# thierrydumas/autoencoder_based_image_compression

Measured on AMD Instinct MI355X. Metric: Mpixels/s encode+decode (Kodak 768x512 luma), bitstream bit-exact, higher is better.
Workload: dtype f32; 1 GPU; kodak_512x768_luma_batch24_per_gpu_bin_width_1.0_lossless_roundtrip; height=512, width=768, truncated_unary_length=10, idx_map_exception=67, parallelism=single GPU, coder=device, 64 maps per wavefront, encode + decode + compare

## Files before the change

autoencoder_based_image_compression_amd/csrc/hip/coder_simd.hip:

```cpp
#include <hip/hip_runtime.h>
#include <stdint.h>

#include <mutex>

#include "../coder/lean_step.h"
#include "eae_hip.h"

int eae_coder_generic_encode(uint32_t n_maps, uint32_t map_size, const int16_t* symbols, uint8_t L, const double* probs,
                             const int32_t* prob_row, uint8_t* streams, uint64_t stride, uint32_t* bac_bits,
                             uint32_t* bypass_bits, int32_t* status, int32_t* stage, int only_status, hipStream_t stream);
int eae_coder_generic_decode(uint32_t n_maps, uint32_t map_size, int16_t* out, uint8_t L, const double* probs,
                             const int32_t* prob_row, const uint8_t* streams, uint64_t stride, const uint32_t* bac_bits,
                             const uint32_t* bypass_bits, int32_t* status, int32_t* stage, int only_status, hipStream_t stream);

#ifndef EAE_RES_BINARISE
#define EAE_RES_BINARISE 47
#endif
#ifndef EAE_RES_ENCODE_CORE
#define EAE_RES_ENCODE_CORE 55
#endif
#ifndef EAE_RES_EMIT
#define EAE_RES_EMIT 39
#endif
#ifndef EAE_RES_DECODE_CORE
#define EAE_RES_DECODE_CORE 55
#endif
#ifndef EAE_RES_DEBINARISE
#define EAE_RES_DEBINARISE 23
#endif
#ifndef EAE_RES_DEBINARISE_STAGED
#define EAE_RES_DEBINARISE_STAGED 39
#endif
#ifndef EAE_RES_DECODE_CORE_CHUNKED
#define EAE_RES_DECODE_CORE_CHUNKED 63
#endif
#ifndef EAE_DECODE_TOPUP_ZEROS
#define EAE_KEEP_VGPR_FREE_(n) asm volatile("; v" #n " reserved: the last register of the allocation holds no operand" ::: "v" #n)
#define EAE_KEEP_LAST_VGPR_FREE(n) EAE_KEEP_VGPR_FREE_(n)
#else
#define EAE_KEEP_LAST_VGPR_FREE(n)
#endif

namespace {

using namespace eae_core;
using namespace eae_lean;


#ifndef EAE_SIMD_PRIO
#define EAE_SIMD_PRIO 3
#endif

constexpr int32_t RETRY = -100;
constexpr uint32_t kMaxFastL = 32;
constexpr uint32_t kRecordPad = 12;
constexpr uint32_t kRing = 32;
constexpr uint32_t kBypassStage = 512;
constexpr uint32_t kDebinariseStage = 1024;
constexpr uint32_t kEmitWords = 224;

struct SimdParams {
    uint32_t n_maps, map_size, L, dcap;
    uint32_t rcap;
    const int16_t* symbols;
    int16_t* decoded;
    const double* probs;
    const int32_t* prob_row;
    uint8_t* streams;
    uint64_t stride;
    uint32_t* bac_bits;
    uint32_t* bypass_bits;
    int32_t* status;
    int32_t* stage;
    uint8_t* decisions;
    uint32_t* ndec;
    uint32_t* records;
    uint8_t* prefixes;
    uint32_t chunk, nchunks;
    uint32_t* group_steps;
    uint2* enc_state;
    uint4* emit_state;
    uint32_t* avail_bits;
    uint4* dec_state;
    uint2* dec_state2;
};

__host__ __device__ inline uint32_t chunk_span(uint32_t steps, uint32_t nchunks) {
    const uint32_t span = ((steps + nchunks - 1u) / nchunks + 63u) & ~63u;
    return span ? span : 64u;
}

__device__ __forceinline__ uint32_t wave_exclusive_scan(uint32_t v, uint32_t& total) {
    int inc = (int)v;
    inc += __builtin_amdgcn_update_dpp(0, inc, 0x111, 0xF, 0xF, false);
    inc += __builtin_amdgcn_update_dpp(0, inc, 0x112, 0xF, 0xF, false);
    inc += __builtin_amdgcn_update_dpp(0, inc, 0x114, 0xF, 0xF, false);
    inc += __builtin_amdgcn_update_dpp(0, inc, 0x118, 0xF, 0xF, false);
    inc += __builtin_amdgcn_update_dpp(0, inc, 0x142, 0xA, 0xF, false);
    inc += __builtin_amdgcn_update_dpp(0, inc, 0x143, 0xC, 0xF, false);
    total = (uint32_t)__builtin_amdgcn_readlane(inc, 63);
    return (uint32_t)inc - v;
}
__device__ __forceinline__ int wave_exclusive_max(int v) {
    int m = __builtin_amdgcn_update_dpp(-1, v, 0x138, 0xF, 0xF, false);
#define EAE_MAX_STEP(ctrl_, rows_)                                                        \
    {                                                                                     \
        const int o_ = __builtin_amdgcn_update_dpp(-1, m, ctrl_, rows_, 0xF, false);      \
        m = o_ > m ? o_ : m;                                                              \
    }
    EAE_MAX_STEP(0x111, 0xF)
    EAE_MAX_STEP(0x112, 0xF)
    EAE_MAX_STEP(0x114, 0xF)
    EAE_MAX_STEP(0x118, 0xF)
    EAE_MAX_STEP(0x142, 0xA)
    EAE_MAX_STEP(0x143, 0xC)
#undef EAE_MAX_STEP
    return m;
}
__device__ __forceinline__ uint32_t wave_max(uint32_t v) {
#pragma unroll
    for (int d = 32; d >= 1; d >>= 1) {
        const uint32_t o = __shfl_xor(v, d, 64);
        v = o > v ? o : v;
    }
    return v;
}

__global__ __launch_bounds__(64) void binarise_kernel(const SimdParams p) {
    EAE_KEEP_LAST_VGPR_FREE(EAE_RES_BINARISE);
    __shared__ unsigned long long ybuf[40];
    const uint32_t m = blockIdx.x, lane = threadIdx.x;
    const int32_t row = p.prob_row ? p.prob_row[m] : (int32_t)m;
    if (row < 0) {
        if (lane == 0) { p.ndec[m] = 0; p.bac_bits[m] = 0; p.bypass_bits[m] = 0; p.status[m] = 0; if (p.stage) p.stage[m] = 0; }
        return;
    }
    const uint32_t L = p.L;
    const int16_t* in = p.symbols + (size_t)m * p.map_size;
    uint8_t* dec = p.decisions + (size_t)(m >> 6) * 64u * p.dcap + (size_t)(m & 63u) * 8u;
    unsigned long long* ystream = reinterpret_cast<unsigned long long*>(p.streams + (uint64_t)m * p.stride + p.stride / 2);
    const uint32_t size_bits = round_up_to_byte(required_bits(p.map_size, L));
    uint32_t jbase = 0, bbase = 0;
    bool overflow = false;
    if (lane < 40) ybuf[lane] = 0;
    for (uint32_t t = 0; t < p.map_size; t += 64) {
        const uint32_t i = t + lane;
        const bool valid = i < p.map_size;
        const int s = valid ? (int)in[i] : 0;
        const uint32_t a = (uint32_t)(s < 0 ? -s : s);
        const uint32_t ones = a < L ? a : L;
        const uint32_t nd = valid ? ones + (a < L ? 1u : 0u) : 0u;
        unsigned long long bb = 0;
        uint32_t nb = 0;
        if (valid && a >= L) {
            const uint32_t v = a - L + 1u;
            const uint32_t n = count_nb_bits(v) - 1u;
            bb = ((1ull << n) - 1ull) | ((unsigned long long)(n ? rev16(v - (1u << n)) >> (16u - n) : 0u) << (n + 1u));
            nb = 2u * n + 1u;
        }
        if (valid && s != 0) {
            bb |= (unsigned long long)(s > 0 ? 1u : 0u) << nb;
            nb++;
        }
        uint32_t both_tot;
        const uint32_t both = wave_exclusive_scan(nd | (nb << 16), both_tot);
        const uint32_t jo = both & 0xFFFFu, bo = both >> 16, jtot = both_tot & 0xFFFFu, btot = both_tot >> 16;
        for (uint32_t q = 0; q < nd; q++) {
            const uint32_t j = jbase + jo + q;
            dec[(size_t)(j >> 3) * 512u + (j & 7u)] = (uint8_t)((q << 1) | (q < ones ? 1u : 0u));
        }
        if (nb) {
            const uint32_t pos = (bbase & 63u) + bo;
            atomicOr(&ybuf[pos >> 6], bb << (pos & 63u));
            if ((pos & 63u) + nb > 64u) atomicOr(&ybuf[(pos >> 6) + 1u], bb >> (64u - (pos & 63u)));
        }
        if (bbase + btot > size_bits) overflow = true;
        if (overflow) break;
        const uint32_t nfull = ((bbase & 63u) + btot) >> 6;
        const unsigned long long mine = lane < 40 ? ybuf[lane] : 0ull;
        const unsigned long long carry = ybuf[nfull];
        if (lane < nfull) ystream[(bbase >> 6) + lane] = mine;
        if (lane < 40) ybuf[lane] = lane == 0 ? carry : 0ull;
        jbase += jtot;
        bbase += btot;
    }
    if (lane == 0) {
        if (!overflow && (bbase & 63u)) ystream[bbase >> 6] = ybuf[0];
        p.ndec[m] = jbase;
        p.bypass_bits[m] = bbase;
        p.bac_bits[m] = 0;
        p.status[m] = overflow ? RETRY : 0;
        if (p.stage) p.stage[m] = 0;
    }
}

extern __shared__ double lds_dyn[];

template <bool CHUNKED>
__global__ __launch_bounds__(64) void bac_encode_core_kernel(const SimdParams p) {
    EAE_KEEP_LAST_VGPR_FREE(EAE_RES_ENCODE_CORE);
    __builtin_amdgcn_s_setprio(EAE_SIMD_PRIO);
    const uint32_t lane = threadIdx.x;
    const uint32_t m = blockIdx.x * 64u + lane;
    const bool in_range = m < p.n_maps;
    const int32_t row = in_range ? (p.prob_row ? p.prob_row[m] : (int32_t)m) : -1;
    const bool live = in_range && row >= 0 && p.status[m] == 0;
    const uint32_t L = p.L;
    double* probs = lds_dyn;
    bool retry = false;
    if (live)
        for (uint32_t k = 0; k < L; k++) {
            const double pk = p.probs[(size_t)row * L + k];
            probs[k * 64u + lane] = scale_probability(pk);
            if (!(pk > 0. && pk < 1.)) retry = true;
        }
    const uint32_t nd = live && !retry ? p.ndec[m] : 0u;
    uint32_t steps = wave_max(nd);
    const uint32_t nd_all = ~wave_max(~(nd ? nd : 0xFFFFFFFFu));
    const uint8_t* dec = p.decisions + (size_t)blockIdx.x * 64u * p.dcap + (size_t)lane * 8u;
    uint32_t* rec = p.records + (size_t)(in_range ? m : 0u) * p.rcap;
    Interval s = interval_init();
    uint32_t j_first = 0;
    if (CHUNKED) {
        if (p.chunk == 0u) { if (lane == 0u) p.group_steps[blockIdx.x] = steps; }
        else steps = p.group_steps[blockIdx.x];
        const uint32_t span = chunk_span(steps, p.nchunks);
        j_first = p.chunk * span < steps ? p.chunk * span : steps;
        steps = j_first + span < steps ? j_first + span : steps;
        if (p.chunk != 0u && in_range) { const uint2 st = p.enc_state[m]; s.lo = st.x; s.hc = st.y; }
    }
    const uint32_t last_round = (steps ? steps - 1u : 0u) >> 3;
    auto decisions_of = [&](uint32_t round) __attribute__((always_inline)) {
        return *reinterpret_cast<const uint2*>(dec + (size_t)(round < last_round ? round : last_round) * 512u);
    };
    uint32_t* const sink = rec + p.dcap + 8u;
    const uint32_t nd_here = CHUNKED ? (nd < steps ? nd : steps) : nd;
    auto round_of_eight = [&](const uint2& d, uint32_t jb) __attribute__((always_inline)) {
        const unsigned long long d8 = (unsigned long long)d.x | ((unsigned long long)d.y << 32);
        auto probability = [&](uint32_t q) __attribute__((always_inline)) {
// ... 348 lines not shown
                    const bool need = rcount <= 32u;
                    rwin |= (unsigned long long)(need ? wnext : 0u) << (need ? 32u - rcount : 0u);
                    rcount += need ? 32u : 0u;
                    rword += need ? 1u : 0u;
                    const DecodeStep d = decode_step(s, code32, pk);
                    const uint32_t k = d.take < left ? d.take : left;
                    uint32_t bits = (uint32_t)((rwin >> 1) >> (63u - k));
                    const uint32_t ext = d.take - k;
                    bits = (bits << ext) | ((bits & 1u) ? ((1u << ext) - 1u) : 0u);
                    rwin <<= k;
                    rcount -= k;
                    left -= k;
                    code32 = shift_code(code32, d, bits);
                    const bool done = !d.one || unary + 1u == L;
                    if (done) prefix[i] = (uint8_t)(d.one ? L : unary);
                    i += done ? 1u : 0u;
                    unary = done ? 0u : unary + 1u;
                    pk = done ? p0 : pspec;
                }
            }
            }
            if (!__any(i < size && (!CHUNKED || final_chunk || (begun && left >= kStepMargin)))) break;
        }
    }
    if (CHUNKED && size && !final_chunk) {
        p.dec_state[m] = make_uint4(s.lo, s.hc, code32, begun ? nbac - left : kNotStarted);
        p.dec_state2[m] = make_uint2(unary, i);
    }
    if (live && retry) p.status[m] = RETRY;
#ifdef EAE_HWID_PROBE
    {
        const unsigned int hw1 = __builtin_amdgcn_s_getreg(((32 - 1) << 11) | (0 << 6) | 4);
        const unsigned int xcc1 = __builtin_amdgcn_s_getreg(((4 - 1) << 11) | (0 << 6) | 20);
        if (lane == 0) {
            atomicAdd(&g_hwid_probe[0], 1u);
            if (((hw1 ^ probe_hw0) & 0xFFFFu) != 0u || xcc1 != probe_xcc0) {
                atomicAdd(&g_hwid_probe[1], 1u);
                g_hwid_probe[2] = probe_hw0; g_hwid_probe[3] = probe_xcc0; g_hwid_probe[4] = hw1; g_hwid_probe[5] = xcc1;
            }
        }
    }
#endif
}

#ifdef EAE_HWID_PROBE
extern "C" int eae_hip_debug_hwid_probe(unsigned int* out8) {
    return (int)hipMemcpyFromSymbol(out8, HIP_SYMBOL(g_hwid_probe), 8 * sizeof(unsigned int));
}
#endif

template <bool STAGED>
__global__ __launch_bounds__(64) void debinarise_kernel(const SimdParams p) {
    if (STAGED) { EAE_KEEP_LAST_VGPR_FREE(EAE_RES_DEBINARISE_STAGED); } else { EAE_KEEP_LAST_VGPR_FREE(EAE_RES_DEBINARISE); }
    __shared__ uint32_t ytile[80];
    const uint32_t m = blockIdx.x, lane = threadIdx.x;
    const int32_t row = p.prob_row ? p.prob_row[m] : (int32_t)m;
    if (lane == 0 && p.ndec) p.ndec[m] = 0u;
    if (row < 0 || p.status[m] != 0) {
        if (row >= 0 && p.status[m] == RETRY && lane == 0 && p.ndec) p.ndec[m] = 1u;
        return;
    }
    const uint32_t L = p.L, size = p.map_size;
    const uint32_t nbyp = p.bypass_bits[m];
    const uint32_t* gbyp = reinterpret_cast<const uint32_t*>(p.streams + (uint64_t)m * p.stride + p.stride / 2);
    const uint32_t ywords = (nbyp + 31u) >> 5;
    const uint8_t* prefix = p.prefixes + (size_t)m * size;
    const int16_t* expected = p.symbols ? p.symbols + (size_t)m * size : nullptr;
    int16_t* out = p.decoded ? p.decoded + (size_t)m * size : nullptr;
    uint32_t ybase = 0;
    bool bad = false, differ = false;
    __shared__ uint32_t ystage[STAGED ? kBypassStage + 80u : 1u];
    __shared__ uint8_t pstage[STAGED ? kDebinariseStage : 1u];
    __shared__ int16_t estage[STAGED ? kDebinariseStage : 1u];
    if (STAGED) {
        const uint32_t have = ywords < kBypassStage ? ywords : kBypassStage, last = ywords ? ywords - 1u : 0u;
        for (uint32_t k = 0; k < have; k += 512u) {
            uint32_t v[8];
#pragma unroll
            for (uint32_t u = 0; u < 8; u++) {
                const uint32_t w = k + u * 64u + lane;
                v[u] = gbyp[w < last ? w : last];
            }
#pragma unroll
            for (uint32_t u = 0; u < 8; u++) {
                const uint32_t w = k + u * 64u + lane;
                if (w < kBypassStage) ystage[w] = w < ywords ? v[u] : 0u;
            }
        }
        for (uint32_t w = have + lane; w < kBypassStage + 80u; w += 64u) ystage[w] = 0u;
    }
    for (uint32_t t = 0; t < size; t += 64u) {
        if (STAGED && (t & (kDebinariseStage - 1u)) == 0u) {
            const uint32_t last = size - 1u;
            __syncthreads();
            for (uint32_t k = 0; k < kDebinariseStage && t + k < size; k += 512u) {
                uint8_t pv[8];
                int16_t ev[8];
#pragma unroll
                for (uint32_t u = 0; u < 8; u++) {
                    const uint32_t i = t + k + u * 64u + lane, at_i = i < last ? i : last;
                    pv[u] = prefix[at_i];
                    ev[u] = expected ? expected[at_i] : (int16_t)0;
                }
#pragma unroll
                for (uint32_t u = 0; u < 8; u++) {
                    pstage[k + u * 64u + lane] = pv[u];
                    estage[k + u * 64u + lane] = ev[u];
                }
            }
            __syncthreads();
        }
        const uint32_t w0 = ybase >> 5;
        const bool in_stage = STAGED && (ywords <= kBypassStage ? w0 <= kBypassStage : w0 + 80u <= kBypassStage);
        if (!in_stage) {
            ytile[lane] = w0 + lane < ywords ? gbyp[w0 + lane] : 0u;
            if (lane < 16u) ytile[64u + lane] = w0 + 64u + lane < ywords ? gbyp[w0 + 64u + lane] : 0u;
        }
        const uint32_t* const window = in_stage ? ystage + w0 : ytile;
        auto bits_at = [&](uint32_t pos) {
            const uint32_t rel = pos - (w0 << 5), q = rel >> 5, sh = rel & 31u;
            const unsigned long long two = (unsigned long long)window[q] | ((unsigned long long)window[q + 1u] << 32);
            return (uint32_t)(two >> sh);
        };
        const uint32_t i = t + lane;
        const bool valid = i < size;
        uint32_t a = valid ? (uint32_t)(STAGED ? pstage[i & (kDebinariseStage - 1u)] : prefix[i]) : 0u;
        const bool nonzero = a != 0u;
        uint32_t ntot;
        uint32_t at = wave_exclusive_scan(nonzero ? 1u : 0u, ntot);
        uint32_t extra = 0;
        unsigned long long escapes = __ballot(valid && a == L);
        uint32_t extra_tot = 0;
        while (escapes) {
            const int e = __builtin_ctzll(escapes);
            escapes &= escapes - 1ull;
            const uint32_t pos = ybase + (uint32_t)__builtin_amdgcn_readlane((int)at, e) + extra_tot;
            const uint32_t w = bits_at(pos);
            const uint32_t nn = (uint32_t)__builtin_ctz(~w | 0x80000000u);
            if (nn > 16u || pos + 2u * nn + 1u > nbyp) { bad = true; break; }
            const uint32_t suffix = nn ? __builtin_bitreverse32(bits_at(pos + nn + 1u)) >> (32u - nn) : 0u;
            const uint32_t value = (L + ((suffix + (1u << nn) - 1u) & 0xFFFFu)) & 0xFFFFu;
            const uint32_t len = 2u * nn + 1u;
            if ((int)lane == e) a = value;
            if ((int)lane >= e) extra += len;
            extra_tot += len;
        }
        if (bad) break;
        const uint32_t spos = ybase + at + extra;
        if (nonzero && spos >= nbyp) bad = true;
        if (__any(bad)) { bad = true; break; }
        int v = (int)(int16_t)a;
        if (nonzero && !(bits_at(spos) & 1u)) v = -v;
        if (valid) {
            if (out) out[i] = (int16_t)v;
            if (expected && (STAGED ? estage[i & (kDebinariseStage - 1u)] : expected[i]) != (int16_t)v) differ = true;
        }
        ybase += ntot + extra_tot;
    }
    const bool any_differ = __any(differ);
    if (lane == 0) {
        if (bad) { p.status[m] = RETRY; if (p.ndec) p.ndec[m] = 1u; }
        else if (expected && any_differ) p.status[m] = MISMATCH;
    }
}

__global__ __launch_bounds__(64) void compare_kernel(const SimdParams p) {
    const uint32_t m = blockIdx.x, lane = threadIdx.x;
    if (p.ndec[m] == 0u) return;
    const int32_t row = p.prob_row ? p.prob_row[m] : (int32_t)m;
    if (row < 0 || p.status[m] != 0) return;
    const int16_t* a = p.symbols + (size_t)m * p.map_size;
    const int16_t* b = p.decoded + (size_t)m * p.map_size;
    int differ = 0;
    for (uint32_t i = lane; i < p.map_size; i += 64) differ |= (a[i] != b[i]);
    if (__any(differ) && lane == 0) p.status[m] = MISMATCH;
}

#ifdef EAE_EXPERIMENTAL_CODER
constexpr uint32_t kPipeRecords = 64u;
constexpr uint32_t kPipeSpinLimit = 1u << 21;
constexpr uint32_t kPipeDone = 0x80000000u, kPipeBad = 0x40000000u;

#define EAE_PIPE_ORDER() asm volatile("s_waitcnt lgkmcnt(0)" ::: "memory")

constexpr size_t pipe_lds_bytes(uint32_t L) {
    return ((size_t)L + 1u) * 64u * sizeof(double) + ((size_t)kPipeRecords + kRing) * 64u * sizeof(uint32_t) + (8u + 4u * 64u) * sizeof(uint32_t);
}

#ifndef EAE_RES_PIPE
#define EAE_RES_PIPE 63
#endif

#ifdef EAE_PIPE_PROBE
__device__ unsigned long long g_pipe_probe[3][4];
__device__ unsigned long long g_pipe_probe2[8];
#define PIPE_T0() const long long probe_t0 = clock64(); long long probe_wait = 0, probe_mark = 0; unsigned probe_rounds = 0
#define PIPE_WAIT_BEGIN() probe_mark = clock64()
#define PIPE_WAIT_END() probe_wait += clock64() - probe_mark
#define PIPE_ROUND() probe_rounds++
#define PIPE_REPORT(role_) if (blockIdx.x == 0 && lane == 0) { g_pipe_probe[role_][0] = clock64() - probe_t0; g_pipe_probe[role_][1] = probe_wait; \
    g_pipe_probe[role_][2] = probe_rounds; g_pipe_probe[role_][3] = __builtin_amdgcn_s_getreg(((32 - 1) << 11) | (0 << 6) | 4); }
#else
#define PIPE_T0()
#define PIPE_WAIT_BEGIN()
#define PIPE_WAIT_END()
#define PIPE_ROUND()
#define PIPE_REPORT(role_)
#endif

// ... 405 lines not shown
        p.prefixes = reinterpret_cast<uint8_t*>(p.records);
    }
    return p;
}

static int check_simd_layout(uint32_t map_size, uint8_t L, const uint8_t* streams, uint64_t stride) {
    const uint64_t half = stride / 2;
    return (half < (uint64_t)(round_up_to_byte(required_bits(map_size, L)) >> 3) + 16 || (stride & 15u) ||
            (reinterpret_cast<uintptr_t>(streams) & 15u)) ? 1 : 0;
}

int eae_hip_coder_encode_batch(uint32_t n_maps, uint32_t map_size, const int16_t* symbols, uint8_t L, const double* probs,
                               const int32_t* prob_row, uint8_t* streams, uint64_t stride, uint32_t* bac_bits,
                               uint32_t* bypass_bits, int32_t* status, int32_t* stage, void* workspace,
                               uint64_t workspace_bytes, void* stream) {
    if (!symbols || !probs || !streams || !bac_bits || !bypass_bits || !status || !workspace) return -1;
    if (check_simd_layout(map_size, L, streams, stride)) return 1;
    if (workspace_bytes < eae_hip_coder_workspace_bytes(n_maps, map_size, L)) return 1;
    if (n_maps == 0) return 0;
    hipStream_t s = (hipStream_t)stream;
    if (!fast_applies(L) || map_size == 0) {
        (void)hipMemsetAsync(status, 0, (size_t)n_maps * sizeof(int32_t), s);
        return eae_coder_generic_encode(n_maps, map_size, symbols, L, probs, prob_row, streams, stride, bac_bits, bypass_bits,
                                        status, stage, 0, s);
    }
    const SimdParams p = make_params(n_maps, map_size, L, symbols, probs, prob_row, streams, stride, bac_bits, bypass_bits,
                                     status, stage, workspace);
    hipLaunchKernelGGL(binarise_kernel, dim3(n_maps), dim3(64), 0, s, p);
    hipLaunchKernelGGL(bac_encode_core_kernel<false>, dim3((n_maps + 63u) / 64u), dim3(64), (size_t)L * 64u * sizeof(double), s, p);
    hipLaunchKernelGGL(emit_kernel<false>, dim3(n_maps), dim3(64), 0, s, p);
    const int rc = eae_coder_generic_encode(n_maps, map_size, symbols, L, probs, prob_row, streams, stride, bac_bits,
                                            bypass_bits, status, stage, RETRY, s);
    return rc ? rc : (int)hipGetLastError();
}

int eae_hip_coder_decode_batch(uint32_t n_maps, uint32_t map_size, int16_t* symbols_out, const int16_t* expected, uint8_t L,
                               const double* probs, const int32_t* prob_row, const uint8_t* streams, uint64_t stride,
                               const uint32_t* bac_bits, const uint32_t* bypass_bits, int32_t* status, int32_t* stage,
                               void* workspace, uint64_t workspace_bytes, void* stream) {
    if (!probs || !streams || !bac_bits || !bypass_bits || !status) return -1;
    if (!symbols_out && (!expected || !workspace)) return -1;
    const bool have_ws = workspace && workspace_bytes >= eae_hip_coder_workspace_bytes(n_maps, map_size, L);
    if (!symbols_out && !have_ws) return 1;
    if (n_maps == 0) return 0;
    hipStream_t s = (hipStream_t)stream;
    SimdParams p = make_params(n_maps, map_size, L, expected, probs, prob_row, const_cast<uint8_t*>(streams), stride,
                               const_cast<uint32_t*>(bac_bits), const_cast<uint32_t*>(bypass_bits), status, stage,
                               have_ws ? workspace : nullptr);
    if (symbols_out) p.decoded = symbols_out;
    if (!expected) (void)hipMemsetAsync(status, 0, (size_t)n_maps * sizeof(int32_t), s);
    const bool fast = fast_applies(L) && map_size && have_ws && !check_simd_layout(map_size, L, streams, stride);
    if (fast) {
        hipLaunchKernelGGL(bac_decode_core_kernel<false>, dim3((n_maps + 63u) / 64u), dim3(64), decode_lds_bytes(L), s, p);
        if (n_maps <= 256u) hipLaunchKernelGGL(debinarise_kernel<true>, dim3(n_maps), dim3(64), 0, s, p);
        else hipLaunchKernelGGL(debinarise_kernel<false>, dim3(n_maps), dim3(64), 0, s, p);
    } else {
        hipLaunchKernelGGL(mark_kernel, dim3((n_maps + 255u) / 256u), dim3(256), 0, s, p);
    }
    const int rc = eae_coder_generic_decode(n_maps, map_size, p.decoded, L, probs, prob_row, streams, stride, bac_bits,
                                            bypass_bits, status, stage, RETRY, s);
    if (rc) return rc;
    if (expected) {
        if (p.ndec) hipLaunchKernelGGL(compare_kernel, dim3(n_maps), dim3(64), 0, s, p);
        else return 1;
    }
    return (int)hipGetLastError();
}

#if defined(EAE_EXPERIMENTAL_CODER) && !defined(EAE_DECODE_TOPUP_ZEROS)
uint64_t eae_hip_coder_trailing_workspace_bytes(uint32_t n_maps, uint32_t map_size, uint8_t L) {
    const uint64_t groups = ((uint64_t)n_maps + 63u) / 64u;
    return eae_hip_coder_workspace_bytes(n_maps, map_size, L) + round256((uint64_t)n_maps * map_size) + round256(groups * 4u) +
           round256((uint64_t)n_maps * 8u) + round256((uint64_t)n_maps * 16u) + round256((uint64_t)n_maps * 4u) +
           round256((uint64_t)n_maps * 16u) + round256((uint64_t)n_maps * 8u) + 256u;
}

namespace {
struct TrailingStreams {
    hipStream_t emit = nullptr, decode = nullptr;
    hipEvent_t encoded[16] = {}, emitted[16] = {}, start = nullptr, done = nullptr;
    bool complete = false;
};
TrailingStreams* trailing_streams() {
    static TrailingStreams sets[16][4];
    static unsigned next[16] = {0};
    static std::mutex guard;
    int dev = 0;
    if (hipGetDevice(&dev) != hipSuccess || dev < 0 || dev >= 16) return nullptr;
    std::lock_guard<std::mutex> hold(guard);
    TrailingStreams& t = sets[dev][next[dev]++ & 3u];
    if (!t.complete) {
        if (!t.emit && hipStreamCreateWithFlags(&t.emit, hipStreamNonBlocking) != hipSuccess) return nullptr;
        if (!t.decode && hipStreamCreateWithFlags(&t.decode, hipStreamNonBlocking) != hipSuccess) return nullptr;
        for (int i = 0; i < 16; i++) {
            if (!t.encoded[i] && hipEventCreateWithFlags(&t.encoded[i], hipEventDisableTiming) != hipSuccess) return nullptr;
            if (!t.emitted[i] && hipEventCreateWithFlags(&t.emitted[i], hipEventDisableTiming) != hipSuccess) return nullptr;
        }
        if (!t.start && hipEventCreateWithFlags(&t.start, hipEventDisableTiming) != hipSuccess) return nullptr;
        if (!t.done && hipEventCreateWithFlags(&t.done, hipEventDisableTiming) != hipSuccess) return nullptr;
        t.complete = true;
    }
    return &t;
}
int trailing_join(TrailingStreams* t, hipStream_t s, int rc) {
    (void)hipEventRecord(t->emitted[0], t->emit);
    (void)hipStreamWaitEvent(t->decode, t->emitted[0], 0);
    (void)hipEventRecord(t->done, t->decode);
    (void)hipStreamWaitEvent(s, t->done, 0);
// ... 113 lines not shown
```

Measured before the change: 3021 Mpixels/s.

## Vectorise binarise with 4 symbols per lane and LDS-staged 64-bit decision writes

The binarise kernel now loads four int16 symbols per lane with one 64-bit load. It builds each symbol's decision bytes as 64-bit patterns, combining them with atomicOr into an LDS window, then flushes whole 64-bit words to global memory. This replaces the per-byte scattered global stores. A windowed fallback covers the case where one iteration produces more decisions than fit in the window. Separately, the debinarise kernel reuses its loaded bypass tile until the read position moves past it, avoiding a reload on every iteration. The cost is added complexity, more LDS usage and LDS atomics, and a risk to bit-exactness in edge cases.

```diff
diff --git a/autoencoder_based_image_compression_amd/csrc/hip/coder_simd.hip b/autoencoder_based_image_compression_amd/csrc/hip/coder_simd.hip
--- a/autoencoder_based_image_compression_amd/csrc/hip/coder_simd.hip
+++ b/autoencoder_based_image_compression_amd/csrc/hip/coder_simd.hip
@@ -126,9 +126,21 @@
     return v;
 }
 
+constexpr uint32_t kDecisionWindow = 128;
+constexpr uint32_t kBypassTile = 130;
+
+__device__ __forceinline__ unsigned long long binarise_pattern(uint32_t c, uint32_t ones, uint32_t nd) {
+    const uint32_t o = ones > 8u * c ? ones - 8u * c : 0u, n = nd - 8u * c;
+    const unsigned long long lo8 = 0x0101010101010101ull;
+    const unsigned long long v = 0x0E0C0A0806040200ull + (unsigned long long)(16u * c) * lo8 + (o >= 8u ? lo8 : lo8 & ((1ull << (8u * o)) - 1ull));
+    return n >= 8u ? v : v & ((1ull << (8u * n)) - 1ull);
+}
+
 __global__ __launch_bounds__(64) void binarise_kernel(const SimdParams p) {
     EAE_KEEP_LAST_VGPR_FREE(EAE_RES_BINARISE);
-    __shared__ unsigned long long ybuf[40];
+    __shared__ unsigned long long dbuf[kDecisionWindow + 1];
+    __shared__ unsigned long long ybuf[kBypassTile];
+    __shared__ unsigned long long first8[18];
     const uint32_t m = blockIdx.x, lane = threadIdx.x;
     const int32_t row = p.prob_row ? p.prob_row[m] : (int32_t)m;
     if (row < 0) {
@@ -137,54 +149,135 @@
     }
     const uint32_t L = p.L;
     const int16_t* in = p.symbols + (size_t)m * p.map_size;
-    uint8_t* dec = p.decisions + (size_t)(m >> 6) * 64u * p.dcap + (size_t)(m & 63u) * 8u;
+    const bool aligned = (reinterpret_cast<uintptr_t>(in) & 7u) == 0u;
+    unsigned long long* dec = reinterpret_cast<unsigned long long*>(p.decisions + (size_t)(m >> 6) * 64u * p.dcap + (size_t)(m & 63u) * 8u);
     unsigned long long* ystream = reinterpret_cast<unsigned long long*>(p.streams + (uint64_t)m * p.stride + p.stride / 2);
     const uint32_t size_bits = round_up_to_byte(required_bits(p.map_size, L));
     uint32_t jbase = 0, bbase = 0;
     bool overflow = false;
-    if (lane < 40) ybuf[lane] = 0;
-    for (uint32_t t = 0; t < p.map_size; t += 64) {
-        const uint32_t i = t + lane;
-        const bool valid = i < p.map_size;
-        const int s = valid ? (int)in[i] : 0;
-        const uint32_t a = (uint32_t)(s < 0 ? -s : s);
-        const uint32_t ones = a < L ? a : L;
-        const uint32_t nd = valid ? ones + (a < L ? 1u : 0u) : 0u;
-        unsigned long long bb = 0;
-        uint32_t nb = 0;
-        if (valid && a >= L) {
-            const uint32_t v = a - L + 1u;
-            const uint32_t n = count_nb_bits(v) - 1u;
-            bb = ((1ull << n) - 1ull) | ((unsigned long long)(n ? rev16(v - (1u << n)) >> (16u - n) : 0u) << (n + 1u));
-            nb = 2u * n + 1u;
-        }
-        if (valid && s != 0) {
-            bb |= (unsigned long long)(s > 0 ? 1u : 0u) << nb;
-            nb++;
+    for (uint32_t w = lane; w < kDecisionWindow + 1u; w += 64u) dbuf[w] = 0ull;
+    for (uint32_t w = lane; w < kBypassTile; w += 64u) ybuf[w] = 0ull;
+    if (lane < 18u) {
+        const uint32_t n = lane >> 1;
+        first8[lane] = binarise_pattern(0u, (lane & 1u) || n == 0u ? n : n - 1u, n);
+    }
+    for (uint32_t t = 0; t < p.map_size; t += 4u * 64u) {
+        const uint32_t i0 = t + 4u * lane;
+        uint2 sw = make_uint2(0u, 0u);
+        if (aligned && i0 + 4u <= p.map_size) {
+            sw = *reinterpret_cast<const uint2*>(in + i0);
+        } else {
+            const uint32_t h[4] = {i0 < p.map_size ? (uint16_t)in[i0] : 0u, i0 + 1u < p.map_size ? (uint16_t)in[i0 + 1u] : 0u,
+                                   i0 + 2u < p.map_size ? (uint16_t)in[i0 + 2u] : 0u, i0 + 3u < p.map_size ? (uint16_t)in[i0 + 3u] : 0u};
+            sw = make_uint2(h[0] | (h[1] << 16), h[2] | (h[3] << 16));
+        }
+        auto sym = [&](uint32_t q) __attribute__((always_inline)) { return (int)(int16_t)((q < 2u ? sw.x : sw.y) >> (16u * (q & 1u))); };
+        uint32_t ndl = 0, nbl = 0, nz = 0;
+#pragma unroll
+        for (uint32_t q = 0; q < 4; q++) {
+            const int sq = sym(q);
+            const uint32_t a = (uint32_t)(sq < 0 ? -sq : sq);
+            ndl += i0 + q < p.map_size ? (a < L ? a + 1u : L) : 0u;
+            nbl += (a >= L ? 2u * (31u - (uint32_t)__builtin_clz(a - L + 1u)) + 1u : 0u) + (sq != 0 ? 1u : 0u);
+            nz |= sq != 0 ? 1u << q : 0u;
         }
         uint32_t both_tot;
-        const uint32_t both = wave_exclusive_scan(nd | (nb << 16), both_tot);
-        const uint32_t jo = both & 0xFFFFu, bo = both >> 16, jtot = both_tot & 0xFFFFu, btot = both_tot >> 16;
-        for (uint32_t q = 0; q < nd; q++) {
-            const uint32_t j = jbase + jo + q;
-            dec[(size_t)(j >> 3) * 512u + (j & 7u)] = (uint8_t)((q << 1) | (q < ones ? 1u : 0u));
-        }
-        if (nb) {
-            const uint32_t pos = (bbase & 63u) + bo;
-            atomicOr(&ybuf[pos >> 6], bb << (pos & 63u));
-            if ((pos & 63u) + nb > 64u) atomicOr(&ybuf[(pos >> 6) + 1u], bb >> (64u - (pos & 63u)));
-        }
-        if (bbase + btot > size_bits) overflow = true;
-        if (overflow) break;
-        const uint32_t nfull = ((bbase & 63u) + btot) >> 6;
-        const unsigned long long mine = lane < 40 ? ybuf[lane] : 0ull;
-        const unsigned long long carry = ybuf[nfull];
-        if (lane < nfull) ystream[(bbase >> 6) + lane] = mine;
-        if (lane < 40) ybuf[lane] = lane == 0 ? carry : 0ull;
+        const uint32_t both = wave_exclusive_scan(ndl | (nbl << 16), both_tot);
+        const uint32_t jtot = both_tot & 0xFFFFu, btot = both_tot >> 16;
+        if (bbase + btot > size_bits) { overflow = true; break; }
+        const uint32_t dstart = jbase & 7u, dend = dstart + jtot, bstart = bbase & 63u;
+        if (dend <= 8u * kDecisionWindow) {
+            uint32_t dat = dstart + (both & 0xFFFFu), bat = bstart + (both >> 16);
+            for (uint32_t left = nz; left != 0u; left &= left - 1u) {
+                const uint32_t q = (uint32_t)__builtin_ctz(left);
+                const int sq = sym(q);
+                const uint32_t a = (uint32_t)(sq < 0 ? -sq : sq);
+                const uint32_t ones = a < L ? a : L, nd = a < L ? a + 1u : L;
+                const uint32_t pos = dat + q, n8 = nd < 8u ? nd : 8u;
+                auto put = [&](uint32_t at, unsigned long long v) __attribute__((always_inline)) {
+                    const uint32_t sh = 8u * (at & 7u);
+                    atomicOr(&dbuf[at >> 3], v << sh);
+                    if (sh) atomicOr(&dbuf[(at >> 3) + 1u], v >> (64u - sh));
+                };
+                put(pos, first8[2u * n8 + ((ones < 8u ? ones : 8u) == n8 ? 1u : 0u)]);
+                for (uint32_t c = 1; 8u * c < nd; c++) put(pos + 8u * c, binarise_pattern(c, ones, nd));
+                dat += nd - 1u;
+                uint32_t nb = 1u;
+                if (a >= L) {
+                    const uint32_t v = a - L + 1u;
+                    const uint32_t n = count_nb_bits(v) - 1u;
+                    const unsigned long long bb = ((1ull << n) - 1ull) | ((unsigned long long)(n ? rev16(v - (1u << n)) >> (16u - n) : 0u) << (n + 1u))
+                                                  | ((unsigned long long)(sq > 0 ? 1u : 0u) << (2u * n + 1u));
+                    nb = 2u * n + 2u;
+                    atomicOr(&ybuf[bat >> 6], bb << (bat & 63u));
+                    if ((bat & 63u) + nb > 64u) atomicOr(&ybuf[(bat >> 6) + 1u], bb >> (64u - (bat & 63u)));
+                } else if (sq > 0) {
+                    atomicOr(&ybuf[bat >> 6], 1ull << (bat & 63u));
+                }
+                bat += nb;
+            }
+            const uint32_t nfull = dend >> 3;
+            for (uint32_t w = lane; w < nfull; w += 64u) dec[(size_t)((jbase >> 3) + w) * 64u] = dbuf[w];
+            const unsigned long long carry = dbuf[nfull];
+            for (uint32_t w = lane; w <= nfull; w += 64u) dbuf[w] = 0ull;
+            if (lane == 0) dbuf[0] = carry;
+        } else for (uint32_t w0 = 0;; w0 += 8u * kDecisionWindow) {
+            uint32_t dat = dstart + (both & 0xFFFFu), bat = bstart + (both >> 16);
+            for (uint32_t left = nz; left != 0u; left &= left - 1u) {
+                const uint32_t q = (uint32_t)__builtin_ctz(left);
+                const int sq = sym(q);
+                const uint32_t a = (uint32_t)(sq < 0 ? -sq : sq);
+                const uint32_t ones = a < L ? a : L, nd = a < L ? a + 1u : L;
+                for (uint32_t c = 0; 8u * c < nd; c++) {
+                    const int rel = (int)(dat + q + 8u * c) - (int)w0;
+                    if (rel >= 8 * (int)kDecisionWindow) break;
+                    if (rel <= -8) continue;
+                    const unsigned long long v = binarise_pattern(c, ones, nd);
+                    const int lo = rel >> 3;
+                    const uint32_t sh = 8u * ((uint32_t)rel & 7u);
+                    if (lo >= 0) atomicOr(&dbuf[lo], v << sh);
+                    if (sh && lo + 1 < (int)kDecisionWindow) atomicOr(&dbuf[lo + 1], v >> (64u - sh));
+                }
+                dat += nd - 1u;
+                if (w0 == 0u) {
+                    unsigned long long bb = 0;
+                    uint32_t nb = 0;
+                    if (a >= L) {
+                        const uint32_t v = a - L + 1u;
+                        const uint32_t n = count_nb_bits(v) - 1u;
+                        bb = ((1ull << n) - 1ull) | ((unsigned long long)(n ? rev16(v - (1u << n)) >> (16u - n) : 0u) << (n + 1u));
+                        nb = 2u * n + 1u;
+                    }
+                    bb |= (unsigned long long)(sq > 0 ? 1u : 0u) << nb;
+                    nb++;
+                    atomicOr(&ybuf[bat >> 6], bb << (bat & 63u));
+                    if ((bat & 63u) + nb > 64u) atomicOr(&ybuf[(bat >> 6) + 1u], bb >> (64u - (bat & 63u)));
+                    bat += nb;
+                }
+            }
+            const uint32_t rem = dend - w0;
+            const uint32_t nfull = rem >> 3 < kDecisionWindow ? rem >> 3 : kDecisionWindow;
+            for (uint32_t w = lane; w < nfull; w += 64u) dec[(size_t)((jbase >> 3) + (w0 >> 3) + w) * 64u] = dbuf[w];
+            if (rem <= 8u * kDecisionWindow) {
+                const unsigned long long carry = dbuf[nfull];
+                for (uint32_t w = lane; w <= nfull; w += 64u) dbuf[w] = 0ull;
+                if (lane == 0) dbuf[0] = carry;
+                break;
+            }
+            for (uint32_t w = lane; w < kDecisionWindow; w += 64u) dbuf[w] = 0ull;
+        }
+        if (btot != 0u) {
+            const uint32_t nfull = (bstart + btot) >> 6;
+            for (uint32_t w = lane; w < nfull; w += 64u) ystream[(bbase >> 6) + w] = ybuf[w];
+            const unsigned long long carry = ybuf[nfull];
+            for (uint32_t w = lane; w <= nfull; w += 64u) ybuf[w] = 0ull;
+            if (lane == 0) ybuf[0] = carry;
+        }
         jbase += jtot;
         bbase += btot;
     }
     if (lane == 0) {
+        if (!overflow && (jbase & 7u)) dec[(size_t)(jbase >> 3) * 64u] = dbuf[0];
         if (!overflow && (bbase & 63u)) ystream[bbase >> 6] = ybuf[0];
         p.ndec[m] = jbase;
         p.bypass_bits[m] = bbase;
@@ -655,6 +748,7 @@
     const int16_t* expected = p.symbols ? p.symbols + (size_t)m * size : nullptr;
     int16_t* out = p.decoded ? p.decoded + (size_t)m * size : nullptr;
     uint32_t ybase = 0;
+    uint32_t wbase = ~0u;
     bool bad = false, differ = false;
     __shared__ uint32_t ystage[STAGED ? kBypassStage + 80u : 1u];
     __shared__ uint8_t pstage[STAGED ? kDebinariseStage : 1u];
@@ -699,13 +793,15 @@
         }
         const uint32_t w0 = ybase >> 5;
         const bool in_stage = STAGED && (ywords <= kBypassStage ? w0 <= kBypassStage : w0 + 80u <= kBypassStage);
-        if (!in_stage) {
+        if (!in_stage && (wbase == ~0u || w0 > wbase + 10u)) {
+            wbase = w0;
             ytile[lane] = w0 + lane < ywords ? gbyp[w0 + lane] : 0u;
             if (lane < 16u) ytile[64u + lane] = w0 + 64u + lane < ywords ? gbyp[w0 + 64u + lane] : 0u;
         }
         const uint32_t* const window = in_stage ? ystage + w0 : ytile;
+        const uint32_t wfirst = in_stage ? w0 : wbase;
         auto bits_at = [&](uint32_t pos) {
-            const uint32_t rel = pos - (w0 << 5), q = rel >> 5, sh = rel & 31u;
+            const uint32_t rel = pos - (wfirst << 5), q = rel >> 5, sh = rel & 31u;
             const unsigned long long two = (unsigned long long)window[q] | ((unsigned long long)window[q + 1u] << 32);
             return (uint32_t)(two >> sh);
         };
```

New measurement: 3042 Mpixels/s (median of 6 runs). No clear change (+0.7%).

## Process four symbols per lane in binarise and debinarise with LDS-staged decision windows

Applied to the files above, without the earlier changes.

Binarise now loads four int16 symbols per lane as one 64-bit load, computes magnitudes and counts with packed 16-bit SIMD ops, and builds decision bytes and bypass bits in LDS windows that are flushed as whole 64-bit words. This replaces the per-byte scattered decision stores and the per-64-symbol scan. Debinarise handles 256 symbols per iteration with one packed scan and a bypass tile sized to need. When only comparison is requested, the decoded-output write is skipped. The trade-off is more complex control flow, extra atomics into LDS, and more register pressure.

```diff
diff --git a/autoencoder_based_image_compression_amd/csrc/hip/coder_simd.hip b/autoencoder_based_image_compression_amd/csrc/hip/coder_simd.hip
--- a/autoencoder_based_image_compression_amd/csrc/hip/coder_simd.hip
+++ b/autoencoder_based_image_compression_amd/csrc/hip/coder_simd.hip
@@ -56,7 +56,10 @@
 constexpr uint32_t kRecordPad = 12;
 constexpr uint32_t kRing = 32;
 constexpr uint32_t kBypassStage = 512;
+constexpr uint32_t kBypassTile = 276;
 constexpr uint32_t kDebinariseStage = 1024;
+constexpr uint32_t kDecisionWindow = 64;
+constexpr uint32_t kBypassWindow = 32;
 constexpr uint32_t kEmitWords = 224;
 
 struct SimdParams {
@@ -126,65 +129,168 @@
     return v;
 }
 
+struct __attribute__((packed, aligned(2))) FourSymbols { unsigned long long v; };
+
 __global__ __launch_bounds__(64) void binarise_kernel(const SimdParams p) {
     EAE_KEEP_LAST_VGPR_FREE(EAE_RES_BINARISE);
-    __shared__ unsigned long long ybuf[40];
+    __shared__ unsigned long long dbuf[kDecisionWindow + 1];
+    __shared__ unsigned long long ybuf[kBypassWindow + 1];
     const uint32_t m = blockIdx.x, lane = threadIdx.x;
     const int32_t row = p.prob_row ? p.prob_row[m] : (int32_t)m;
     if (row < 0) {
         if (lane == 0) { p.ndec[m] = 0; p.bac_bits[m] = 0; p.bypass_bits[m] = 0; p.status[m] = 0; if (p.stage) p.stage[m] = 0; }
         return;
     }
-    const uint32_t L = p.L;
-    const int16_t* in = p.symbols + (size_t)m * p.map_size;
-    uint8_t* dec = p.decisions + (size_t)(m >> 6) * 64u * p.dcap + (size_t)(m & 63u) * 8u;
+    const uint32_t L = p.L, size = p.map_size;
+    const int16_t* in = p.symbols + (size_t)m * size;
+    unsigned long long* dstream = reinterpret_cast<unsigned long long*>(p.decisions + (size_t)(m >> 6) * 64u * p.dcap + (size_t)(m & 63u) * 8u);
     unsigned long long* ystream = reinterpret_cast<unsigned long long*>(p.streams + (uint64_t)m * p.stride + p.stride / 2);
-    const uint32_t size_bits = round_up_to_byte(required_bits(p.map_size, L));
+    const uint32_t size_bits = round_up_to_byte(required_bits(size, L));
     uint32_t jbase = 0, bbase = 0;
     bool overflow = false;
-    if (lane < 40) ybuf[lane] = 0;
-    for (uint32_t t = 0; t < p.map_size; t += 64) {
-        const uint32_t i = t + lane;
-        const bool valid = i < p.map_size;
-        const int s = valid ? (int)in[i] : 0;
-        const uint32_t a = (uint32_t)(s < 0 ? -s : s);
-        const uint32_t ones = a < L ? a : L;
-        const uint32_t nd = valid ? ones + (a < L ? 1u : 0u) : 0u;
-        unsigned long long bb = 0;
-        uint32_t nb = 0;
-        if (valid && a >= L) {
-            const uint32_t v = a - L + 1u;
-            const uint32_t n = count_nb_bits(v) - 1u;
-            bb = ((1ull << n) - 1ull) | ((unsigned long long)(n ? rev16(v - (1u << n)) >> (16u - n) : 0u) << (n + 1u));
-            nb = 2u * n + 1u;
-        }
-        if (valid && s != 0) {
-            bb |= (unsigned long long)(s > 0 ? 1u : 0u) << nb;
-            nb++;
+    dbuf[lane] = 0ull;
+    if (lane <= kBypassWindow) ybuf[lane] = 0ull;
+    if (lane == 0) dbuf[kDecisionWindow] = 0ull;
+    const uint32_t last4 = size >= 4u ? size - 4u : 0u;
+    auto load_tiny = [&]() __attribute__((always_inline)) {
+        unsigned long long v = 0ull;
+#pragma unroll
+        for (uint32_t q = 0; q < 4; q++) v |= (unsigned long long)(uint16_t)in[4u * lane + q < size ? 4u * lane + q : size - 1u] << (16u * q);
+        return v;
+    };
+    const FourSymbols* const four_at = size >= 4u ? reinterpret_cast<const FourSymbols*>(in) : reinterpret_cast<const FourSymbols*>(p.probs);
+    const uint32_t four_step = size >= 4u ? 2u : 0u;
+    auto load_four = [&](uint32_t t) __attribute__((always_inline)) {
+        const uint32_t i0 = t + 4u * lane;
+        return reinterpret_cast<const FourSymbols*>(reinterpret_cast<const uint8_t*>(four_at) + (size_t)(i0 < last4 ? i0 : last4) * four_step)->v;
+    };
+    auto own_four = [&](unsigned long long loaded, uint32_t t) __attribute__((always_inline)) {
+        const uint32_t i0 = t + 4u * lane, skip = i0 > last4 ? i0 - last4 : 0u;
+        return size < 4u ? loaded : loaded >> (16u * (skip < 3u ? skip : 3u));
+    };
+    typedef short pair_i16 __attribute__((ext_vector_type(2)));
+    typedef unsigned short pair_u16 __attribute__((ext_vector_type(2)));
+    const uint32_t LL = L | (L << 16);
+    auto magnitudes = [](uint32_t two) __attribute__((always_inline)) {
+        const pair_i16 minus = __builtin_bit_cast(pair_i16, (pair_u16)(0) - __builtin_bit_cast(pair_u16, two));
+        return __builtin_bit_cast(uint32_t, __builtin_elementwise_max(__builtin_bit_cast(pair_i16, two), minus));
+    };
+    auto decision_counts = [&](uint32_t a2) __attribute__((always_inline)) {
+        const pair_u16 one = (pair_u16)(1);
+        return __builtin_bit_cast(uint32_t, __builtin_elementwise_min(__builtin_bit_cast(pair_u16, a2) + one, __builtin_bit_cast(pair_u16, LL)));
+    };
+    auto nonzeros = [](uint32_t a2) __attribute__((always_inline)) {
+        return __builtin_bit_cast(uint32_t, __builtin_elementwise_min(__builtin_bit_cast(pair_u16, a2), (pair_u16)(1)));
+    };
+    auto halves = [](uint32_t two) __attribute__((always_inline)) { return (two & 0xFFFFu) + (two >> 16); };
+    auto escape_bits = [&](uint32_t a, unsigned long long& bb) __attribute__((always_inline)) {
+        const uint32_t v = a - L + 1u;
+        const uint32_t n = count_nb_bits(v) - 1u;
+        bb = ((1ull << n) - 1ull) | ((unsigned long long)(n ? rev16(v - (1u << n)) >> (16u - n) : 0u) << (n + 1u));
+        return 2u * n + 1u;
+    };
+    constexpr uint32_t kDone = 0x80000000u;
+    unsigned long long ahead = size >= 4u ? load_four(0u) : load_tiny();
+    for (uint32_t t = 0; t < size; t += 256u) {
+        unsigned long long four = own_four(ahead, t);
+        ahead = load_four(t + 256u);
+        uint32_t pad = 0;
+        if (t + 256u > size) {
+            const uint32_t i0 = t + 4u * lane;
+            const uint32_t nvalid = i0 < size ? (size - i0 < 4u ? size - i0 : 4u) : 0u;
+            four &= nvalid == 4u ? ~0ull : (1ull << (16u * nvalid)) - 1ull;
+            pad = t + 256u - size;
+        }
+        uint32_t sums;
+        {
+            const uint32_t a_lo = magnitudes((uint32_t)four), a_hi = magnitudes((uint32_t)(four >> 32));
+            const pair_u16 nd = __builtin_bit_cast(pair_u16, decision_counts(a_lo)) + __builtin_bit_cast(pair_u16, decision_counts(a_hi));
+            const pair_u16 nz = __builtin_bit_cast(pair_u16, nonzeros(a_lo)) + __builtin_bit_cast(pair_u16, nonzeros(a_hi));
+            sums = halves(__builtin_bit_cast(uint32_t, nd)) | (halves(__builtin_bit_cast(uint32_t, nz)) << 16);
+            const pair_u16 top = __builtin_elementwise_max(__builtin_bit_cast(pair_u16, a_lo), __builtin_bit_cast(pair_u16, a_hi));
+            if (__any((uint32_t)(top.x > top.y ? top.x : top.y) >= L)) {
+#pragma unroll
+                for (uint32_t q = 0; q < 4; q++) {
+                    const uint32_t a = ((q < 2 ? a_lo : a_hi) >> (16u * (q & 1u))) & 0xFFFFu;
+                    unsigned long long bb;
+                    if (a >= L) sums += escape_bits(a, bb) << 16;
+                }
+            }
         }
         uint32_t both_tot;
-        const uint32_t both = wave_exclusive_scan(nd | (nb << 16), both_tot);
-        const uint32_t jo = both & 0xFFFFu, bo = both >> 16, jtot = both_tot & 0xFFFFu, btot = both_tot >> 16;
-        for (uint32_t q = 0; q < nd; q++) {
-            const uint32_t j = jbase + jo + q;
-            dec[(size_t)(j >> 3) * 512u + (j & 7u)] = (uint8_t)((q << 1) | (q < ones ? 1u : 0u));
-        }
-        if (nb) {
-            const uint32_t pos = (bbase & 63u) + bo;
-            atomicOr(&ybuf[pos >> 6], bb << (pos & 63u));
-            if ((pos & 63u) + nb > 64u) atomicOr(&ybuf[(pos >> 6) + 1u], bb >> (64u - (pos & 63u)));
-        }
-        if (bbase + btot > size_bits) overflow = true;
-        if (overflow) break;
-        const uint32_t nfull = ((bbase & 63u) + btot) >> 6;
-        const unsigned long long mine = lane < 40 ? ybuf[lane] : 0ull;
-        const unsigned long long carry = ybuf[nfull];
-        if (lane < nfull) ystream[(bbase >> 6) + lane] = mine;
-        if (lane < 40) ybuf[lane] = lane == 0 ? carry : 0ull;
+        const uint32_t both = wave_exclusive_scan(sums, both_tot);
+        const uint32_t jtot = (both_tot & 0xFFFFu) - pad, btot = both_tot >> 16;
+        if (bbase + btot > size_bits) { overflow = true; break; }
+        const uint32_t dend = (jbase & 7u) + jtot;
+        const uint32_t yend = (bbase & 63u) + btot;
+        uint32_t wd = 0, wy = btot ? 0u : kDone;
+        for (;;) {
+            asm volatile("" : "+v"(four));
+            const uint32_t a_lo = magnitudes((uint32_t)four), a_hi = magnitudes((uint32_t)(four >> 32));
+            const uint32_t nd_lo = decision_counts(a_lo), nd_hi = decision_counts(a_hi);
+            uint32_t pd = (jbase & 7u) + (both & 0xFFFFu), py = (bbase & 63u) + (both >> 16);
+#pragma unroll
+            for (uint32_t q = 0; q < 4; q++) {
+                const uint32_t a = ((q < 2 ? a_lo : a_hi) >> (16u * (q & 1u))) & 0xFFFFu;
+                const uint32_t nd = ((q < 2 ? nd_lo : nd_hi) >> (16u * (q & 1u))) & 0xFFFFu;
+                if (a != 0u) {
+                    for (uint32_t k = 0; k < nd; k += 8u) {
+                        const uint32_t at = pd + k, w = (at >> 3) - wd;
+                        if (w < kDecisionWindow) {
+                            const uint32_t c = nd - k < 8u ? nd - k : 8u;
+                            const unsigned long long piece = (((0x0F0D0B0907050301ull + (unsigned long long)(k >> 3) * 0x1010101010101010ull) << (64u - 8u * c)) >> (64u - 8u * c)) -
+                                                             ((unsigned long long)(a < L && k + 8u >= nd ? 1u : 0u) << (8u * (c - 1u)));
+                            const uint32_t sh = 8u * (at & 7u);
+                            const unsigned long long over = (piece >> 1) >> (63u - sh);
+                            atomicOr(&dbuf[w], piece << sh);
+                            if (over) atomicOr(&dbuf[w + 1u], over);
+                        }
+                    }
+                    const uint32_t positive = ((uint32_t)(four >> (16u * q + 15u)) & 1u) ^ 1u;
+                    const uint32_t w = (py >> 6) - wy, sh = py & 63u;
+                    if (a >= L) {
+                        unsigned long long bb;
+                        uint32_t nb = escape_bits(a, bb);
+                        bb |= (unsigned long long)positive << nb;
+                        nb++;
+                        if (w < kBypassWindow) {
+                            atomicOr(&ybuf[w], bb << sh);
+                            if (sh + nb > 64u) atomicOr(&ybuf[w + 1u], bb >> (64u - sh));
+                        }
+                        py += nb;
+                    } else {
+                        if (w < kBypassWindow) atomicOr(reinterpret_cast<uint32_t*>(ybuf) + 2u * w + (sh >> 5), positive << (sh & 31u));
+                        py += 1u;
+                    }
+                }
+                pd += nd;
+            }
+            if (wd != kDone) {
+                const uint32_t left = (dend >> 3) - wd;
+                const uint32_t nfull = left < kDecisionWindow ? left : kDecisionWindow;
+                const unsigned long long mine = dbuf[lane];
+                const unsigned long long carry = dbuf[nfull];
+                if (lane < nfull) dstream[(size_t)((jbase >> 3) + wd + lane) * 64u] = mine;
+                dbuf[lane] = lane == 0 ? carry : 0ull;
+                if (lane == 0) dbuf[kDecisionWindow] = 0ull;
+                wd = dend <= (wd + kDecisionWindow) * 8u ? kDone : wd + kDecisionWindow;
+            }
+            if (wy != kDone) {
+                const uint32_t left = (yend >> 6) - wy;
+                const uint32_t nfull = left < kBypassWindow ? left : kBypassWindow;
+                const unsigned long long mine = lane <= kBypassWindow ? ybuf[lane] : 0ull;
+                const unsigned long long carry = ybuf[nfull];
+                if (lane < nfull) ystream[(bbase >> 6) + wy + lane] = mine;
+                if (lane <= kBypassWindow) ybuf[lane] = lane == 0 ? carry : 0ull;
+                wy = yend <= (wy + kBypassWindow) * 64u ? kDone : wy + kBypassWindow;
+            }
+            if (wd == kDone && wy == kDone) break;
+        }
         jbase += jtot;
         bbase += btot;
     }
     if (lane == 0) {
+        if (jbase & 7u) dstream[(size_t)(jbase >> 3) * 64u] = dbuf[0];
         if (!overflow && (bbase & 63u)) ystream[bbase >> 6] = ybuf[0];
         p.ndec[m] = jbase;
         p.bypass_bits[m] = bbase;
@@ -639,7 +745,7 @@
 template <bool STAGED>
 __global__ __launch_bounds__(64) void debinarise_kernel(const SimdParams p) {
     if (STAGED) { EAE_KEEP_LAST_VGPR_FREE(EAE_RES_DEBINARISE_STAGED); } else { EAE_KEEP_LAST_VGPR_FREE(EAE_RES_DEBINARISE); }
-    __shared__ uint32_t ytile[80];
+    __shared__ uint32_t ytile[kBypassTile];
     const uint32_t m = blockIdx.x, lane = threadIdx.x;
     const int32_t row = p.prob_row ? p.prob_row[m] : (int32_t)m;
     if (lane == 0 && p.ndec) p.ndec[m] = 0u;
@@ -676,7 +782,7 @@
         }
         for (uint32_t w = have + lane; w < kBypassStage + 80u; w += 64u) ystage[w] = 0u;
     }
-    for (uint32_t t = 0; t < size; t += 64u) {
+    for (uint32_t t = 0; t < size; t += 256u) {
         if (STAGED && (t & (kDebinariseStage - 1u)) == 0u) {
             const uint32_t last = size - 1u;
             __syncthreads();
@@ -697,51 +803,74 @@
             }
             __syncthreads();
         }
+        uint32_t a[4];
+        uint32_t counts = 0;
+#pragma unroll
+        for (uint32_t q = 0; q < 4; q++) {
+            const uint32_t i = t + q * 64u + lane;
+            const uint32_t pv = STAGED ? pstage[i & (kDebinariseStage - 1u)] : prefix[i < size ? i : size - 1u];
+            a[q] = i < size ? pv : 0u;
+            counts |= (a[q] != 0u ? 1u : 0u) << (8u * q);
+        }
+        uint32_t totals;
+        const uint32_t before = wave_exclusive_scan(counts, totals);
+        const uint32_t ntot = (totals & 0xFFu) + ((totals >> 8) & 0xFFu) + ((totals >> 16) & 0xFFu) + (totals >> 24);
+        unsigned long long escapes[4];
+        uint32_t nesc = 0;
+#pragma unroll
+        for (uint32_t q = 0; q < 4; q++) {
+            escapes[q] = __ballot(a[q] == L);
+            nesc += (uint32_t)__builtin_popcountll(escapes[q]);
+        }
         const uint32_t w0 = ybase >> 5;
-        const bool in_stage = STAGED && (ywords <= kBypassStage ? w0 <= kBypassStage : w0 + 80u <= kBypassStage);
-        if (!in_stage) {
-            ytile[lane] = w0 + lane < ywords ? gbyp[w0 + lane] : 0u;
-            if (lane < 16u) ytile[64u + lane] = w0 + 64u + lane < ywords ? gbyp[w0 + 64u + lane] : 0u;
-        }
+        const uint32_t nwin = (((ybase & 31u) + ntot + 33u * nesc) >> 5) + 2u;
+        const bool in_stage = STAGED && w0 + nwin <= (ywords <= kBypassStage ? kBypassStage + 80u : kBypassStage);
+        if (!in_stage)
+            for (uint32_t w = lane; w < nwin; w += 64u) ytile[w] = w0 + w < ywords ? gbyp[w0 + w] : 0u;
         const uint32_t* const window = in_stage ? ystage + w0 : ytile;
         auto bits_at = [&](uint32_t pos) {
             const uint32_t rel = pos - (w0 << 5), q = rel >> 5, sh = rel & 31u;
             const unsigned long long two = (unsigned long long)window[q] | ((unsigned long long)window[q + 1u] << 32);
             return (uint32_t)(two >> sh);
         };
-        const uint32_t i = t + lane;
-        const bool valid = i < size;
-        uint32_t a = valid ? (uint32_t)(STAGED ? pstage[i & (kDebinariseStage - 1u)] : prefix[i]) : 0u;
-        const bool nonzero = a != 0u;
-        uint32_t ntot;
-        uint32_t at = wave_exclusive_scan(nonzero ? 1u : 0u, ntot);
-        uint32_t extra = 0;
-        unsigned long long escapes = __ballot(valid && a == L);
-        uint32_t extra_tot = 0;
-        while (escapes) {
-            const int e = __builtin_ctzll(escapes);
-            escapes &= escapes - 1ull;
-            const uint32_t pos = ybase + (uint32_t)__builtin_amdgcn_readlane((int)at, e) + extra_tot;
-            const uint32_t w = bits_at(pos);
-            const uint32_t nn = (uint32_t)__builtin_ctz(~w | 0x80000000u);
-            if (nn > 16u || pos + 2u * nn + 1u > nbyp) { bad = true; break; }
-            const uint32_t suffix = nn ? __builtin_bitreverse32(bits_at(pos + nn + 1u)) >> (32u - nn) : 0u;
-            const uint32_t value = (L + ((suffix + (1u << nn) - 1u) & 0xFFFFu)) & 0xFFFFu;
-            const uint32_t len = 2u * nn + 1u;
-            if ((int)lane == e) a = value;
-            if ((int)lane >= e) extra += len;
-            extra_tot += len;
+        uint32_t extra_tot = 0, slot_base = 0;
+#pragma unroll
+        for (uint32_t q = 0; q < 4; q++) {
+            if (!bad) {
+                const bool nonzero = a[q] != 0u;
+                const uint32_t at = slot_base + ((before >> (8u * q)) & 0xFFu);
+                uint32_t extra = extra_tot;
+                unsigned long long todo = escapes[q];
+                while (todo) {
+                    const int e = __builtin_ctzll(todo);
+                    todo &= todo - 1ull;
+                    const uint32_t pos = ybase + (uint32_t)__builtin_amdgcn_readlane((int)at, e) + extra_tot;
+                    const uint32_t w = bits_at(pos);
+                    const uint32_t nn = (uint32_t)__builtin_ctz(~w | 0x80000000u);
+                    if (nn > 16u || pos + 2u * nn + 1u > nbyp) { bad = true; break; }
+                    const uint32_t suffix = nn ? __builtin_bitreverse32(bits_at(pos + nn + 1u)) >> (32u - nn) : 0u;
+                    const uint32_t value = (L + ((suffix + (1u << nn) - 1u) & 0xFFFFu)) & 0xFFFFu;
+                    const uint32_t len = 2u * nn + 1u;
+                    if ((int)lane == e) a[q] = value;
+                    if ((int)lane >= e) extra += len;
+                    extra_tot += len;
+                }
+                const uint32_t spos = ybase + at + extra;
+                if (nonzero && spos >= nbyp) bad = true;
+                bad = __any(bad);
+                if (!bad) {
+                    int v = (int)(int16_t)a[q];
+                    if (nonzero && !(bits_at(spos) & 1u)) v = -v;
+                    const uint32_t i = t + q * 64u + lane;
+                    if (i < size) {
+                        if (out) out[i] = (int16_t)v;
+                        if (expected && (STAGED ? estage[i & (kDebinariseStage - 1u)] : expected[i]) != (int16_t)v) differ = true;
+                    }
+                }
+                slot_base += (totals >> (8u * q)) & 0xFFu;
+            }
         }
         if (bad) break;
-        const uint32_t spos = ybase + at + extra;
-        if (nonzero && spos >= nbyp) bad = true;
-        if (__any(bad)) { bad = true; break; }
-        int v = (int)(int16_t)a;
-        if (nonzero && !(bits_at(spos) & 1u)) v = -v;
-        if (valid) {
-            if (out) out[i] = (int16_t)v;
-            if (expected && (STAGED ? estage[i & (kDebinariseStage - 1u)] : expected[i]) != (int16_t)v) differ = true;
-        }
         ybase += ntot + extra_tot;
     }
     const bool any_differ = __any(differ);
@@ -1253,8 +1382,10 @@
     const bool fast = fast_applies(L) && map_size && have_ws && !check_simd_layout(map_size, L, streams, stride);
     if (fast) {
         hipLaunchKernelGGL(bac_decode_core_kernel<false>, dim3((n_maps + 63u) / 64u), dim3(64), decode_lds_bytes(L), s, p);
-        if (n_maps <= 256u) hipLaunchKernelGGL(debinarise_kernel<true>, dim3(n_maps), dim3(64), 0, s, p);
-        else hipLaunchKernelGGL(debinarise_kernel<false>, dim3(n_maps), dim3(64), 0, s, p);
+        SimdParams q = p;
+        if (!symbols_out) q.decoded = nullptr;
+        if (n_maps <= 256u) hipLaunchKernelGGL(debinarise_kernel<true>, dim3(n_maps), dim3(64), 0, s, q);
+        else hipLaunchKernelGGL(debinarise_kernel<false>, dim3(n_maps), dim3(64), 0, s, q);
     } else {
         hipLaunchKernelGGL(mark_kernel, dim3((n_maps + 255u) / 256u), dim3(256), 0, s, p);
     }
```

Result: no change. 3031 Mpixels/s before, 3048 Mpixels/s after, median of 6 (+0.6%).
